# nathanweeks/exonerate

Measured on AMD Instinct MI355X. Metric: DP cells/s (first-pass lattice cells / end-to-end time), est2genome 1kb x 100kb batch, bit-exact vulgar vs reference, higher is better.
Workload: dtype int32 (packed int16 where proven exact)

## Files before the change

### exonerate_amd/csrc/c4_engine.hip

```cpp
#include <hip/hip_runtime.h>

#include <algorithm>
#include <chrono>
#include <cmath>
#include <cstdio>
#include <cstdlib>
#include <cstring>
#include <numeric>
#include <string>
#include <map>
#include <memory>
#include <vector>
#include <thread>
#include <atomic>
#include <mutex>

#include "c4gpu.h"
#include "c4_internal.h"
#include "c4_config.h"
#include "c4_memrule.h"
#include "c4_launch.h"
#include "c4_kernel_choice.h"
#include "c4_sdp_launch.h"
#include "c4_sdp_host.h"

using namespace c4k;

namespace c4h {
static thread_local std::string g_error;
void set_error(const std::string &msg) { g_error = msg; }
}

#define HIP_OK(expr)                                                                           \
    do {                                                                                       \
        hipError_t e_ = (expr);                                                                \
        if (e_ != hipSuccess) {                                                                \
            c4h::set_error(std::string(#expr) + ": " + hipGetErrorString(e_));                 \
            return -1;                                                                         \
        }                                                                                      \
    } while (0)

struct c4gpu_ctx {
    int device = 0;
    hipStream_t stream = nullptr;
    bool owns_stream = false;
// ... 25 lines not shown
```

### exonerate_amd/csrc/c4_engine_launch.inc

```
struct JobSpec {
    int pair;
    c4gpu_region region;
    int first_state = 0, final_state = 1, cp_count = 0;
    int root = 0;
    int first_cell[CELL_MAX] = {0};
    bool dump_checkpoints = false;
    const c4gpu_subopt *sub = nullptr;
    const int32_t *span_in = nullptr;
    int32_t *span_out = nullptr;
};
typedef std::vector<std::pair<int32_t, int32_t>> RegionPoints;
struct RunList {
    static constexpr int INLINE = 6;
    int n = 0;
    uint32_t small[INLINE];
    std::vector<uint32_t> big;
    const uint32_t *begin() const { return n <= INLINE ? small : big.data(); }
    const uint32_t *end() const { return begin() + n; }
    void assign_reversed(const uint32_t *first, int count) {
        n = count;
        uint32_t *dst = small;
        if (count > INLINE) { big.resize(count); dst = big.data(); }
        for (int k = 0; k < count; k++) dst[k] = first[count - 1 - k];
    }
// ... 8 lines not shown

struct SeedPlan {
    int mode = 0;
    int kshift = 11;
    bool fmt16 = false;
    int seedw = 0, dc = 0;
    std::vector<long long> off;
    std::vector<int> rows;
    std::vector<long long> base;
    std::vector<int> d, t0w, t0_base;
    int hops = 0;
};

double splice_best_sum(const c4gpu_splice_model &sp, bool absolute) {
    double sum = 0;
    for (int r = 0; r < sp.model_length && r < C4GPU_SPLICE_MAX_LEN; r++) {
        double mx = 0;
        for (int c = 0; c < 5; c++) mx = std::max(mx, absolute ? std::fabs((double)sp.data[r][c]) : (double)sp.data[r][c]);
        sum += mx;
    }
    return sum;
}

struct Engine {
    c4gpu_ctx *ctx;
    const c4gpu_model *model;
    int family;
    bool local;
    bool local_exact = true;
    bool pk16_params_ok = false;
    double calc_bound = 0;
    int pk16_match_max = 1, pk16_max_intron = 0;
    int pk16_intron_gain = 0, pk16_intron_cols = 4;
    int loop_tr_host[16] = {-1, -1, -1, -1, -1, -1, -1, -1, -1, -1, -1, -1, -1, -1, -1, -1};
    DevBuf<KParams> kparams;
    DevBuf<DevJob> d_jobs;
    DevBuf<DevResult> d_results;
    DevBuf<DevVsa> d_vsa;
    DevBuf<uint32_t> d_runs, d_runs_out;
    DevBuf<unsigned long long> d_runs_used;
    DevBuf<uint8_t> d_ops;
    DevBuf<int> d_bnd, d_ckpt, d_ckpt_dump, d_queue;
    DevBuf<uint32_t> d_tb;
    DevBuf<int> d_sub_t, d_sub_q, d_sub_colptr, d_span, d_seed, d_pairs;
    DevBuf<DevJob> d_fjobs, d_fsub_jobs;
    DevBuf<DevResult> d_fres, d_fsub_res;
    DevBuf<DevVsa> d_fvsa;
    DevBuf<int> d_ffirst, d_fflags, d_fout;
    DevBuf<unsigned long long> d_fstats;
    DevBuf<FusePair> d_fpairs;
    std::vector<DevJob> hf_jobs;
    std::vector<DevResult> hf_res;
    std::vector<int> hf_first, hf_flags, hf_out;
// ... 34 lines not shown
        }
        kp.start_scope = m->start_scope; kp.end_scope = m->end_scope;
        bool protein = false;
        for (int i = 0; i < m->n_calcs; i++)
            if (m->calcs[i].kind == C4GPU_CALC_MATCH_PROTEIN || m->calcs[i].kind == C4GPU_CALC_MATCH_P2D ||
                m->calcs[i].kind == C4GPU_CALC_MATCH_CODON) protein = true;
        memcpy(kp.submat, protein ? &params->protein_submat[0][0] : &params->dna_submat[0][0], sizeof(int) * 24 * 24);
        bool dna_match = false;
        for (int i = 0; i < m->n_calcs; i++) dna_match |= m->calcs[i].kind == C4GPU_CALC_MATCH_DNA;
        const bool veto = annotated && dna_match && !protein;
        for (int c = 0; c < 24; c++) kp.submat[24 * 24 + c] = veto ? C4GPU_IMPOSSIBLY_LOW_SCORE : 0;
        {
            double pmax = 0;
            for (int i = 0; i < m->n_calcs; i++) pmax = std::max(pmax, std::fabs((double)m->calcs[i].value));
            for (int i = 0; i < 24 * 24; i++) pmax = std::max(pmax, std::fabs((double)kp.submat[i]));
            double smax = 0;
            if (family_has_splice(family))
                for (int k = 0; k < 4; k++) smax = std::max(smax, splice_best_sum(params->splice[k], true) + 1.0);
            local_exact = (pmax + smax) * (m->n_states + 4) < 4.0e8;
            calc_bound = pmax + smax;
            double mmax = 0;
            for (int i = 0; i < 24 * 24; i++) mmax = std::max(mmax, (double)kp.submat[i]);
            pk16_match_max = (int)std::max(1.0, mmax);
            pk16_params_ok = pmax <= 16000.0 && smax <= 16000.0 && params->min_intron >= 0 && params->min_intron <= 30000 &&
                             params->max_intron >= params->min_intron;
            pk16_max_intron = params->max_intron;
            if (veto) {
                local_exact = false;
                pk16_params_ok = false;
                calc_bound = std::max(calc_bound, 987654321.0);
            }
            if (family_has_splice(family)) {
                int best[4];
                for (int k = 0; k < 4; k++) best[k] = (int)std::floor(splice_best_sum(params->splice[k], false) + 0.5) + 1;
                long long gain = -0x40000000LL;
                for (int st = 0; st < m->n_states; st++) {
                    long long pre = -0x40000000LL, post = -0x40000000LL;
                    for (int k = 0; k < m->n_transitions; k++) {
                        const c4gpu_transition &t = m->transitions[k];
                        if (t.calc < 0) continue;
                        const c4gpu_calc &cc = m->calcs[t.calc];
                        const int prm = cc.param & 3;
                        if (cc.kind == C4GPU_CALC_SPLICE_PRE && t.output == st) pre = std::max<long long>(pre, (long long)cc.value + best[prm]);
                        if (cc.kind == C4GPU_CALC_SPLICE_POST && t.input == st) post = std::max<long long>(post, (long long)cc.value + best[prm]);
                    }
                    if (pre > -0x40000000LL && post > -0x40000000LL) gain = std::max(gain, pre + post);
                }
                pk16_intron_gain = (int)std::max<long long>(0, std::min<long long>(gain, 1 << 20));
                pk16_intron_cols = std::max(4, params->min_intron);
                const bool loop_on = !(c4cfg::is(c4cfg::LOOP_SHORTCUT, 0));
                bool others_cost = true;
                for (int k = 0; k < m->n_transitions; k++) {
                    const c4gpu_transition &t = m->transitions[k];
                    if (t.advance_query != 0 || t.calc < 0) continue;
                    const c4gpu_calc &cc = m->calcs[t.calc];
                    if (cc.kind == C4GPU_CALC_SPLICE_PRE || cc.kind == C4GPU_CALC_SPLICE_POST) continue;
                    if (cc.kind != C4GPU_CALC_CONST || cc.value > 0) others_cost = false;
                }
                if (loop_on && family == FAM_EST2GENOME && others_cost && m->n_states <= 16) {
                    int tight[4];
                    for (int k = 0; k < 4; k++) tight[k] = (int)std::floor(splice_best_sum(params->splice[k], false) + 0.5 + 1e-3);
                    for (int st = 0; st < m->n_states; st++) {
                        long long pre = -0x40000000LL, post = -0x40000000LL;
                        int loop = -1;
                        bool clean = true;
                        for (int k = 0; k < m->n_transitions; k++) {
                            const c4gpu_transition &t = m->transitions[k];
                            const c4gpu_calc *cc = t.calc >= 0 ? &m->calcs[t.calc] : nullptr;
                            if (t.input == st && t.output == st) {
                                if (t.advance_query == 0 && t.advance_target == 1 && !cc && loop < 0) loop = k; else clean = false;
// ... 13 lines not shown
        }
        for (int i = 0; i < 16; i++) kp.loop_tr[i] = loop_tr_host[i];
        if (c4cfg::has(c4cfg::TRACE) && family == FAM_EST2GENOME) {
            std::string which;
            for (int i = 0; i < 16; i++) if (loop_tr_host[i] >= 0) which += " " + std::to_string(i) + ":" + std::to_string(loop_tr_host[i]);
            fprintf(stderr, "c4gpu trace: one-row sections answered without a DP for states (state:loop transition)%s\n",
                    which.empty() ? " none" : which.c_str());
        }
        for (int c = 0; c < 4096; c++) {
            const uint8_t row = params->submat_index[params->aa[params->trans[c]]];
            kp.codon_row[c] = row < 24 ? row : 0;
        }
        return 0;
    }

    bool cont_free_ok(long long q_plus_t) const {
        if (c4cfg::is(c4cfg::CONT_FREE, 0)) return false;
        return (double)(q_plus_t + 2) * std::max(calc_bound, 1.0) < 4.0e8;
    }

    bool pk16_fits(int query_length, int target_length) const {
        const double gain = (double)(query_length + 1) * pk16_match_max +
                            (double)(target_length / pk16_intron_cols + 1) * pk16_intron_gain;
        return gain <= 16000.0 && (!family_has_splice(family) || (long long)target_length + 4 <= (long long)pk16_max_intron);
    }
    int ensure_ss16(const ResidentSeqs &seqs) {
        if (!family_has_splice(family)) return 0;
        std::lock_guard<std::mutex> hold(seqs.ss16_lock);
        if (!seqs.ss16_built) {
            if (seqs.ss16.alloc((size_t)seqs.ss_len)) return -1;
            HIP_OK(pk16_build_splice(family, kparams.p, seqs.dev.ss, seqs.dev.ss_stride, seqs.ss_len, seqs.ss16.p, ctx->stream));
            HIP_OK(c4_stream_sync(ctx->stream));
            seqs.ss16_built = true;
        }
        return 0;
    }

    int run(const ResidentSeqs &seqs, int mode, bool cont, const std::vector<JobSpec> &specs, std::vector<JobOut> &out,
            SeedPlan *seed = nullptr) {
        const int n = (int)specs.size();
        if (seed) return run_impl(seqs, mode, cont, specs, out, nullptr, seed);
        for (int i = 0; i < n; i++)
            if (specs[i].span_in || specs[i].span_out) return run_impl(seqs, mode, cont, specs, out, nullptr);
        std::vector<int> plain, blocked;
        std::vector<RegionPoints> pts;
        for (int i = 0; i < n; i++) {
            const c4gpu_subopt *so = specs[i].sub ? specs[i].sub : (pair_sub ? (*pair_sub)[specs[i].pair] : nullptr);
// ... 45 lines not shown
        LaunchFacts f;
        f.family = family; f.mode = mode; f.cont = cont; f.n = n; f.blocked = pts != nullptr;
        f.local = local; f.local_exact = local_exact;
        f.starts_pack = mode == MODE_REGION;
        for (int i = 0; i < n && f.starts_pack; i++)
            f.starts_pack = nbits(specs[i].region.query_length) + nbits(specs[i].region.target_length) <= 31;
        for (int i = 0; i < n; i++) {
            const int sp = specs[i].span_in ? 1 : (specs[i].span_out ? 2 : 0);
            if (i && sp != f.span) { c4h::set_error("jobs with and without span matrices in one call"); return -1; }
            f.span = sp;
        }
        const int span = f.span;
        if (cont && (mode == MODE_PATH || mode == MODE_CKPT) && !pts && !span) {
            long long worst = 0;
            bool cells_leave = false;
            for (int i = 0; i < n; i++) {
                worst = std::max(worst, (long long)specs[i].region.query_length + specs[i].region.target_length);
                cells_leave |= specs[i].dump_checkpoints;
            }
            f.cont_free = !cells_leave && cont_free_ok(worst);
        }
        if (seed) { f.seed_mode = seed->mode; f.kshift = seed->kshift; f.fmt16 = seed->fmt16; }
        f.pk16_params_ok = pk16_params_ok;
        f.pk16_all_fit = f.seed_mode == 1;
        for (int i = 0; i < n && f.pk16_all_fit; i++) f.pk16_all_fit = pk16_fits(specs[i].region.query_length, specs[i].region.target_length);
        f.tdense_n = seqs.tdense_n; f.ss16_built = seqs.ss16_built;
        f.cu_count = ctx->prop.multiProcessorCount;
        if (!cont) {
            h_qlen.resize(n);
            for (int i = 0; i < n; i++) h_qlen[i] = specs[i].region.query_length;
            f.query_length = h_qlen.data(); f.n_lengths = n;
        }
        const KernelChoice choice = choose_kernel(f, sw);
        if (choice.error) { c4h::set_error(choice.error); return -1; }
        const KernelInfo *ki = choice.ki;
        if (choice.needs_ss16 && ensure_ss16(seqs)) return -1;
        if (seed) {
            seed->fmt16 = choice.fmt16;
            if (seed->mode == 1) { seed->seedw = ki->seedw; seed->dc = ki->max_at; }
            if (tr.on) fprintf(stderr, "c4gpu trace:   seeded pass %d with kernel %s\n", seed->mode, ki->name);
        }
        const uint8_t *staged_codes = choice.staged_codes ? seqs.tdense.p : nullptr;
        LaunchPlan lp;
        if (plan_jobs(specs, mode, ki, pts, span, seed, tr, lp)) return -1;
        if (launch_jobs(seqs, mode, ki, specs, pts, span, seed, staged_codes, tr, lp)) return -1;
        tr.lap("runs downloaded");
// ... 248 lines not shown
```

### exonerate_amd/csrc/c4_kernel_choice.h

```cpp
#pragma once
#include <algorithm>

#include "c4_config.h"
#include "c4_launch.h"

namespace c4k {

enum Pk16Form : int {
    PK16_ASM = 0,
    PK16_PLAIN = 1,
    PK16_COUNTERS = 2,
    PK16_DUMP16 = 3,
    PK16_STAGED_BARRIER = 4,
    PK16_STAGED = 5,
    PK16_STAGED_NW8 = 6,
    PK16_STAGED_R6 = 7,
    PK16_STAGED_C8 = 8,
    PK16_STAGED_LONG = 9,
    PK16_FORMS
};
enum Win16Shape : int {
    WIN16_R4W2 = 0,
    WIN16_R3W3 = 1, WIN16_R2W4 = 2, WIN16_R6W2 = 3,
    WIN16_R4W2N4 = 4,
// ... 43 lines not shown
        return s;
    }
};

struct LaunchFacts {
    int family = 0, mode = 0;
    bool cont = false;
    int n = 0;
    bool blocked = false;
    int span = 0;
    bool local = false, local_exact = false;
    bool starts_pack = false;
    bool cont_free = false;
    int seed_mode = 0;
    int kshift = 0;
    bool fmt16 = false;
    bool pk16_params_ok = false;
    bool pk16_all_fit = false;
    int tdense_n = 0;
    bool ss16_built = false;
    int cu_count = 0;
    const int *query_length = nullptr;
    int n_lengths = 0;
};

struct KernelChoice {
    const KernelInfo *ki;
    bool fmt16;
    bool needs_ss16;
    bool staged_codes;
    const char *error;
};

inline int window_waves(int family, const Switches &sw) {
    const int nw = sw.win_nw == 2 ? 2 : 4;
    return get_kernel_mw(family, MODE_REGION, true, true, nw, false, 2) ? nw : 4;
}

inline Pk16Form pk16_base_form(const Switches &sw) { return sw.pk16 == 3 ? PK16_ASM : sw.pk16 == 4 ? PK16_COUNTERS : PK16_PLAIN; }

inline bool pk16_enabled(int family, bool pk16_params_ok, long long n_jobs, const Switches &sw) {
    return family == FAM_EST2GENOME && pk16_params_ok && n_jobs >= 2 && sw.pk16 != 0 &&
           get_kernel_pk16(family, pk16_base_form(sw)) != nullptr;
}

inline void choose_pk16(const LaunchFacts &f, const Switches &sw, KernelChoice &c) {
    c.ki = get_kernel_pk16(f.family, pk16_base_form(sw));
    c.needs_ss16 = sw.pk16 != 3;
    if (sw.pk16 != 1 || !sw.win16) return;
    const KernelInfo *kd = get_kernel_pk16(f.family, PK16_DUMP16);
    if (!kd || !get_kernel_win16(f.family, WIN16_R4W2) || f.kshift > 15 || f.tdense_n <= 0) return;
    int rows = 0;
    for (int i = 0; i < f.n_lengths; i++) rows = std::max(rows, f.query_length[i] + 1);
    if (rows > 32000) return;
    c.ki = kd; c.fmt16 = true;
    const KernelInfo *ke = sw.pk16_io ? get_kernel_pk16(f.family, sw.pk16_io == 2 ? PK16_STAGED : PK16_STAGED_BARRIER) : nullptr;
    if (!ke) return;
    const bool counters = sw.pk16_io == 2;
    const bool strips_ok = rows <= pk16_staged_rows();
    if (f.tdense_n > pk16_staged_codes() && f.tdense_n <= 8 && counters && sw.pk16_c8 && strips_ok &&
        get_kernel_pk16(f.family, PK16_STAGED_C8)) {
        c.ki = get_kernel_pk16(f.family, PK16_STAGED_C8); c.staged_codes = true;
    }
    if (f.tdense_n > pk16_staged_codes()) return;
    if (strips_ok) {
        c.ki = ke; c.staged_codes = true;
        const KernelInfo *kg = (counters && sw.pk16_nw8 != 0) ? get_kernel_pk16(f.family, PK16_STAGED_NW8) : nullptr;
        if (kg && (sw.pk16_nw8 == 1 || (f.n + 1) / 2 <= f.cu_count)) c.ki = kg;
    } else if (counters && sw.pk16_r6) {
        const KernelInfo *kh = get_kernel_pk16(f.family, PK16_STAGED_R6), *kj = get_kernel_pk16(f.family, PK16_STAGED_LONG);
        if (kh && rows <= pk16_staged_rows6()) { c.ki = kh; c.staged_codes = true; }
        else if (kj && sw.pk16_long) { c.ki = kj; c.staged_codes = true; }
    }
}

inline KernelChoice choose_kernel(const LaunchFacts &f, const Switches &sw) {
    KernelChoice c{nullptr, f.fmt16, false, false, nullptr};
    const bool rect = !f.cont && (f.mode == MODE_SCORE || f.mode == MODE_REGION);
// ... 46 lines not shown
```

### exonerate_amd/csrc/c4_viterbi16_kernel.h

```cpp
#pragma once
#include "c4_viterbi_kernel.h"

namespace c4k {

typedef short pk_s2 __attribute__((ext_vector_type(2)));
template <int VAR> __device__ __forceinline__ int pk_add(int a, int b) {
    if constexpr (VAR >= 1) return __builtin_bit_cast(int, __builtin_elementwise_add_sat(__builtin_bit_cast(pk_s2, a), __builtin_bit_cast(pk_s2, b)));
    else { int r; asm("v_pk_add_i16 %0, %1, %2 clamp" : "=v"(r) : "v"(a), "v"(b)); return r; }
}
template <int VAR> __device__ __forceinline__ int pk_max(int a, int b) {
    if constexpr (VAR >= 1) return __builtin_bit_cast(int, __builtin_elementwise_max(__builtin_bit_cast(pk_s2, a), __builtin_bit_cast(pk_s2, b)));
    else { int r; asm("v_pk_max_i16 %0, %1, %2" : "=v"(r) : "v"(a), "v"(b)); return r; }
}
__device__ __forceinline__ int pk_sub(int a, int b) { int r; asm("v_pk_sub_i16 %0, %1, %2 clamp" : "=v"(r) : "v"(a), "v"(b)); return r; }
__device__ __forceinline__ int pk_neg_mask(int d, int fifteen) { int r; asm("v_pk_ashrrev_i16 %0, %1, %2" : "=v"(r) : "v"(fifteen), "v"(d)); return r; }
template <int VAR> __device__ __forceinline__ int pk_lt_mask(int a, int b, int fifteen) {
    if constexpr (VAR >= 1) {
        int r;
        asm("v_pk_sub_i16 %0, %1, %2 clamp\n\tv_pk_ashrrev_i16 %0, 15, %0 op_sel_hi:[0,1]" : "=&v"(r) : "v"(a), "v"(b));
        return r;
    } else {
        return pk_neg_mask(pk_sub(a, b), fifteen);
    }
}
__device__ __forceinline__ int pk_pack(int lo, int hi) { return (int)__builtin_amdgcn_perm((unsigned)hi, (unsigned)lo, 0x05040100u); }
__device__ __forceinline__ int pk_half(int x, int h) { return h ? (x >> 16) : ((x << 16) >> 16); }
__device__ __forceinline__ int clamp16(int x) { return x < -32768 ? -32768 : (x > 32767 ? 32767 : x); }

constexpr int NEG16 = (int)0x80008000u;


template <class M>
struct Dump16 {
    using W1 = WaveDP<M, 1, MODE_SCORE, false, true, false, false, 0, 1>;
    static constexpr bool live(int s) { return M::NDES > 0 && W1::slot_live(s, 0); }
    static constexpr bool inner(int s) { return s != M::START && s != M::END; }
    static constexpr int n_inner() { int n = 0; for (int s = 0; s < M::NS; s++) n += inner(s); return n; }
    static constexpr int n_live() { int n = 0; for (int s = 0; s < M::NS; s++) n += (inner(s) && live(s)); return n; }
    static constexpr int NH = n_inner() + n_live();
    static constexpr int SEEDW16 = (NH + 1) / 2;
    static constexpr int half_of_sc(int s) { int n = 0; for (int x = 0; x < s; x++) n += inner(x); return n; }
    static constexpr int half_of_il(int s) { int n = n_inner(); for (int x = 0; x < s; x++) n += (inner(x) && live(x)); return n; }
    static constexpr int state_of_half(int h) {
        if (h < n_inner()) { for (int s = 0; s < M::NS; s++) if (inner(s) && half_of_sc(s) == h) return s; return -1; }
        for (int s = 0; s < M::NS; s++) if (inner(s) && live(s) && half_of_il(s) == h) return s;
        return -1;
    }
};

template <class M, int R, int VAR = 0, bool DUMP16 = false, int IO = 0, int NCODE_ = 6, bool MEMC = false>
struct WaveDP16 {
    using F = Facts<M>;
    static_assert(M::MAXAQ == 1, "the packed forms exchange exactly one query row per step");
    using W32 = WaveDP<M, R, MODE_SCORE, false, true, false, false, 0, 1>;
    using D16 = Dump16<M>;
    static constexpr int NS = M::NS, NCOL = M::MAXAT + 1, W = 64 * R, DC = M::MAXAT, SEEDW = DUMP16 ? D16::SEEDW16 : W32::SEEDW;
    static constexpr bool live(int s) { return M::NDES > 0 && W32::slot_live(s, 0); }
    static constexpr int NEXP = F::n_exported();
    static constexpr int n_exported_live() { int n = 0; for (int x = 0; x < NS; x++) n += (F::exported(x) && live(x)); return n; }
    static constexpr int BND = IO ? (NEXP + n_exported_live() + 3) / 4 * 4 : NEXP * 2;
    static constexpr int RING = 256;
    static constexpr int CH = IO ? 63 / NCOL * NCOL : (64 + NCOL - 1) / NCOL * NCOL;
    static constexpr int NCODE = NCODE_;
    static constexpr int STAGE_COLS = 128, STAGE_INTS = 8;
    static constexpr int NP = (R + 1) / 2, PROF_EB = (R == 6) ? 12 : 8, PROF_CODE = 64 * PROF_EB;
    static constexpr int PROF_INTS = NCODE * PROF_CODE / 4;
    static_assert(!IO || (VAR >= 1 && F::has_splice() && (R == 6 || R == 4 || R == 2)), "the staged form is built for the packed splice entries and 2, 4 or 6 rows per lane");
    static_assert(!F::has_phase(), "split-codon calcs are not packed");
    static_assert(M::NDES <= 1, "one shadow designation");
    typedef __attribute__((address_space(3))) int lds_int;
    struct C16 { int sc[NS]; int il[NS]; };
    __device__ __forceinline__ static lds_int *lds_at(int a) { return (lds_int *)(size_t)(unsigned)a; }
    __device__ __forceinline__ static int lds_addr(const lds_int *p) { return (int)(unsigned)(size_t)p; }

    const KParams *kp;
    int lane;
    const uint8_t *qc[2], *tc[2];
    const int *ss[2];
    const uint2 *ss16[2];
    long long ss_stride;
// ... 79 lines not shown
    __device__ __forceinline__ void prefetch_profile() {
        const lds_int *pa = lds_at(prof_a[0] + nx_off[0]), *pb = lds_at(prof_a[1] + nx_off[1]);
        static_for<NP>([&](auto K_) __attribute__((always_inline)) { constexpr int K = K_; nx_prof[K] = pa[K]; nx_prof[3 + K] = pb[K]; });
    }
    __device__ __forceinline__ void fill_stage(lds_int *stage, int c0) {
        constexpr int mat = F::match_at();
        const int c = c0 + lane;
        uint2 sv[2]; int off[2];
        static_for<2>([&](auto H_) __attribute__((always_inline)) { constexpr int H = H_;
            int ti = t0[H] + c - mat;
            ti = ti < 0 ? 0 : (ti > tlast[H] ? tlast[H] : ti);
            int tp = t0[H] + c - 2;
            tp = tp < 0 ? 0 : (tp > tlast[H] ? tlast[H] : tp);
            sv[H] = ss16[H][(unsigned)tp];
            off[H] = (int)tdense[tc[H][(unsigned)ti]] * PROF_CODE;
        });
        lds_int *p = stage + (c & (STAGE_COLS - 1));
        p[0 * STAGE_COLS] = (int)__builtin_amdgcn_perm(sv[1].x, sv[0].x, 0x05040100u);
        p[1 * STAGE_COLS] = (int)__builtin_amdgcn_perm(sv[1].x, sv[0].x, 0x07060302u);
        p[2 * STAGE_COLS] = (int)__builtin_amdgcn_perm(sv[1].y, sv[0].y, 0x05040100u);
        p[3 * STAGE_COLS] = (int)__builtin_amdgcn_perm(sv[1].y, sv[0].y, 0x07060302u);
        p[4 * STAGE_COLS] = off[0]; p[5 * STAGE_COLS] = off[1];
    }
    static constexpr int DEAD_ROW = -16000;
    __device__ __forceinline__ void build_profile(int i0) {
        static_for<2>([&](auto H_) __attribute__((always_inline)) { constexpr int H = H_;
            int qr[R];
            static_for<R>([&](auto RR_) __attribute__((always_inline)) { constexpr int RR = RR_;
                const int i = i0 + RR;
                qr[RR] = 24 * ((i >= 1 && i <= Q[H]) ? (int)qc[H][q0[H] + i - 1] : 0);
            });
            for (int d = 0; d < NCODE; d++) {
                const int code = tdense[24 + d];
                int v[R];
                static_for<R>([&](auto RR_) __attribute__((always_inline)) { constexpr int RR = RR_;
                    v[RR] = (i0 + RR > Q[H]) ? DEAD_ROW : clamp16(kp->submat[qr[RR] + code]);
                });
                lds_int *p = lds_at(prof_a[H] + d * PROF_CODE);
                static_for<NP>([&](auto K_) __attribute__((always_inline)) { constexpr int K = K_; p[K] = pk_pack(v[2 * K], v[2 * K + 1 < R ? 2 * K + 1 : 2 * K]); });
            }
        });
    }

    __device__ __forceinline__ void prefetch_column(int j) {
        if constexpr (IO == 1) { prefetch_staged(); return; }
        constexpr int mat = F::match_at();
        static_for<2>([&](auto H_) __attribute__((always_inline)) { constexpr int H = H_;
            int ti = t0[H] + j - mat;
            ti = ti < 0 ? 0 : (ti > tlast[H] ? tlast[H] : ti);
            nx_tcode[H] = tc[H][(unsigned)ti];
            if constexpr (F::has_splice()) {
                int tp = t0[H] + j - 2;
                tp = tp < 0 ? 0 : (tp > tlast[H] ? tlast[H] : tp);
                if constexpr (VAR >= 1) {
                    nx_sp16[H] = ss16[H][(unsigned)tp];
                } else {
                    static_for<4>([&](auto K_) __attribute__((always_inline)) { constexpr int K = K_;
                        nx_sp[H][K] = ss[H][(long long)K * ss_stride + tp];
                    });
                }
            }
        });
    }

    template <int RR, int PH, bool JINT>
    __device__ __forceinline__ void eval_cell(int j, int ms, const int (&sp)[4]) {
        C16 &c = col[PH][RR];
        static_for<M::NT>([&](auto K_) __attribute__((always_inline)) { constexpr int K = K_;
            constexpr TrDesc t = M::tr[K];
            constexpr int PD = (PH - t.at + NCOL) % NCOL;
            const C16 &src = (t.aq == 0) ? col[PD][RR] : (RR > 0 ? col[PD][RR > 0 ? RR - 1 : 0] : nbr[PD]);
            int cand;
            if constexpr (t.in == M::START) cand = 0;
            else cand = src.sc[t.in];
            if constexpr (t.calc >= 0) {
                constexpr CalcDesc cd = M::calc[t.calc];
                if constexpr (cd.kind == CALC_CONST) cand = pk_add<VAR>(cand, cv_pk[t.calc]);
                else if constexpr (cd.kind >= CALC_MATCH_DNA && cd.kind <= CALC_MATCH_P2D) cand = pk_add<VAR>(cand, ms);
                else if constexpr (cd.kind == CALC_SPLICE_PRE) cand = pk_add<VAR>(cand, sp[cd.param]);
                else if constexpr (cd.kind == CALC_SPLICE_POST) {
                    static_assert(live(t.in), "post-splice calc without a length");
                    const int bad = pk_neg_mask(src.il[t.in], fifteen);
                    const int sv = (bad & NEG16) | (~bad & sp[cd.param]);
                    cand = pk_add<VAR>(cand, sv);
                }
            }
            if constexpr (!JINT && t.at > 0) cand = (j >= t.at) ? cand : NEG16;
            int ilc = 0;
            if constexpr (live(t.out)) {
                if constexpr (F::owns_shadow(t.in, 0)) ilc = open_il_pk;
                else if constexpr (live(t.in)) ilc = pk_add<VAR>(src.il[t.in], at_pk[t.at]);
            }
            if constexpr (F::code(K) == 1) {
                c.sc[t.out] = cand;
                if constexpr (live(t.out)) c.il[t.out] = ilc;
            } else {
                if constexpr (live(t.out)) {
                    const int win = pk_lt_mask<VAR>(c.sc[t.out], cand, fifteen);
                    c.il[t.out] = (win & ilc) | (~win & c.il[t.out]);
                }
                c.sc[t.out] = pk_max<VAR>(c.sc[t.out], cand);
            }
        });
    }

    template <bool JINT, int PH>
    __device__ __forceinline__ void step(int s, int i0, bool last_strip, const int *bnd_in, int *bnd_out) {
        const int j = s - lane;
        int ms[R];
        if constexpr (IO == 1) {
            static_for<NP>([&](auto K_) __attribute__((always_inline)) { constexpr int K = K_;
                ms[2 * K] = (int)__builtin_amdgcn_perm((unsigned)nx_prof[3 + K], (unsigned)nx_prof[K], 0x05040100u);
                if constexpr (2 * K + 1 < R) ms[2 * K + 1] = (int)__builtin_amdgcn_perm((unsigned)nx_prof[3 + K], (unsigned)nx_prof[K], 0x07060302u);
            });
        } else {
            static_for<R>([&](auto RR_) __attribute__((always_inline)) { constexpr int RR = RR_;
                ms[RR] = pk_pack(kp->submat[qrow[0][RR] + nx_tcode[0]], kp->submat[qrow[1][RR] + nx_tcode[1]]);
            });
// ... 6 lines not shown
            sp[1] = (int)__builtin_amdgcn_perm(nx_sp16[1].x, nx_sp16[0].x, 0x07060302u);
            sp[2] = (int)__builtin_amdgcn_perm(nx_sp16[1].y, nx_sp16[0].y, 0x05040100u);
            sp[3] = (int)__builtin_amdgcn_perm(nx_sp16[1].y, nx_sp16[0].y, 0x07060302u);
        } else if constexpr (F::has_splice()) {
            static_for<M::NC>([&](auto CI_) __attribute__((always_inline)) { constexpr int CI = CI_;
                constexpr CalcDesc cd = M::calc[CI];
                if constexpr (cd.kind == CALC_SPLICE_PRE)
                    sp[cd.param] = pk_pack(clamp16(kp->calc_value[CI] + nx_sp[0][cd.param]), clamp16(kp->calc_value[CI] + nx_sp[1][cd.param]));
                if constexpr (cd.kind == CALC_SPLICE_POST)
                    sp[cd.param] = pk_pack(clamp16(nx_sp[0][cd.param]), clamp16(nx_sp[1][cd.param]));
            });
        }
        for_exported([&](auto S_, int) __attribute__((always_inline)) { constexpr int S = S_;
            nbr[PH].sc[S] = dpp_shr1(nx_carry.sc[S], expo.sc[S]);
            if constexpr (live(S)) nbr[PH].il[S] = dpp_shr1(nx_carry.il[S], expo.il[S]);
        });
        prefetch_carry(s + 1, bnd_in);
        prefetch_column(j + 1);
        static_for<R>([&](auto RR_) __attribute__((always_inline)) { constexpr int RR = RR_;
            eval_cell<RR, PH, JINT>(j, ms[RR], sp);
            if constexpr (IO == 1 && RR == R / 2 - 1) prefetch_profile();
        });
        {
            int m = col[PH][0].sc[M::END];
            static_for<R>([&](auto RR_) __attribute__((always_inline)) { constexpr int RR = RR_; if constexpr (RR > 0) m = pk_max<VAR>(m, col[PH][RR].sc[M::END]); });
            const bool cand = (pk_sub(best_pk, m) & NEG16) != 0;
            if (__builtin_amdgcn_ballot_w64(cand)) {
                static_for<2>([&](auto H_) __attribute__((always_inline)) { constexpr int H = H_;
                    const bool jact = (j >= 0) & (j <= T[H]);
                    static_for<R>([&](auto RR_) __attribute__((always_inline)) { constexpr int RR = RR_;
                        const int tsc = pk_half(col[PH][RR].sc[M::END], H);
                        const bool upd = jact & (i0 + RR <= Q[H]) & (!best_set[H] | (best[H] < tsc));
                        int from = -1, fsc = 0;
                        static_for<M::NT>([&](auto K_) __attribute__((always_inline)) { constexpr int K = K_;
                            constexpr TrDesc t = M::tr[K];
                            if constexpr (t.out == M::END && t.in != M::START) {
                                const int v = pk_half(col[PH][RR].sc[t.in], H);
                                const bool win = (from < 0) | (fsc < v);
                                fsc = win ? v : fsc;
                                from = win ? t.in : from;
                            }
                        });
                        best[H] = upd ? tsc : best[H];
                        best_i[H] = upd ? (((i0 + RR) << 4) | from) : best_i[H];
                        best_j[H] = upd ? j : best_j[H];
                        best_set[H] = best_set[H] | upd;
                    });
                });
                best_pk = pk_pack(best_set[0] ? best[0] : pk_half(unset_pk, 0), best_set[1] ? best[1] : pk_half(unset_pk, 1));
            }
        }
        for_exported([&](auto S_, int) __attribute__((always_inline)) { constexpr int S = S_;
            expo.sc[S] = col[PH][R - 1].sc[S];
            if constexpr (live(S)) expo.il[S] = col[PH][R - 1].il[S];
        });
        if constexpr (IO == 1) {
            if (lane == 63 && (JINT || (j >= 0 && j <= Tm))) {
                bool to_memory = false;
                if constexpr (MEMC) to_memory = mem_out;
                if (to_memory) {
                    int *p = bnd_out + (long long)j * BND;
                    for_exported([&](auto S_, int slot) __attribute__((always_inline)) { constexpr int S = S_;
                        p[slot] = expo.sc[S];
                        if constexpr (live(S)) p[slot + 1] = expo.il[S];
                    });
                } else {
                    lds_int *p = ring_out + (j & ring_out_mask) * BND;
                    for_exported([&](auto S_, int slot) __attribute__((always_inline)) { constexpr int S = S_;
                        p[slot] = expo.sc[S];
                        if constexpr (live(S)) p[slot + 1] = expo.il[S];
                    });
                }
// ... 6 lines not shown
                    if constexpr (live(S)) p[1] = expo.il[S];
                });
            } else {
                for_exported([&](auto S_, int slot) __attribute__((always_inline)) { constexpr int S = S_;
                    int *p = bnd_out + (long long)j * BND + slot;
                    p[0] = expo.sc[S];
                    if constexpr (live(S)) p[1] = expo.il[S];
                });
            }
        }
        if (((unsigned)(s + DC - 1) & (unsigned)((1 << seed_kshift) - 1)) <= (unsigned)(DC + 62)) {
            const int d = (j + DC - 1) >> seed_kshift;
            const unsigned which = (unsigned)(j - ((d << seed_kshift) - (DC - 1)));
            static_for<2>([&](auto H_) __attribute__((always_inline)) { constexpr int H = H_;
                if ((j >= 0) & (j <= T[H]) & (d >= 1) & (which < (unsigned)DC) & ((d << seed_kshift) <= T[H])) {
                    static_for<R>([&](auto RR_) __attribute__((always_inline)) { constexpr int RR = RR_;
                        const int i = i0 + RR;
                        if (i <= Q[H]) {
                            int *p = seed_wr[H] + (((long long)(d - 1) * DC + which) * seed_rows[H] + i) * SEEDW;
                            if constexpr (DUMP16) {
                                auto half_reg = [&](auto HI_) __attribute__((always_inline)) -> int { constexpr int HI = HI_;
                                    constexpr int S = D16::state_of_half(HI);
                                    if constexpr (S < 0) return 0;
                                    else if constexpr (HI < D16::n_inner()) return col[PH][RR].sc[S];
                                    else return pk_add<VAR>(col[PH][RR].il[S], lim_pk);
                                };
                                static_for<D16::SEEDW16>([&](auto K_) __attribute__((always_inline)) { constexpr int K = K_;
                                    const int va = half_reg(IC<2 * K>{}), vb = half_reg(IC<2 * K + 1>{});
                                    store_dword<K * 4>(p, (int)__builtin_amdgcn_perm((unsigned)vb, (unsigned)va, H ? 0x07060302u : 0x05040100u));
                                });
                            } else {
                                static_for<NS>([&](auto S_) __attribute__((always_inline)) { constexpr int S = S_;
                                    store_dword<S * 4>(p, pk_half(col[PH][RR].sc[S], H));
                                    if constexpr (live(S))
                                        store_dword<W32::dump_pos(S, 0) * 4>(p, t0[H] + j - pk_half(pk_add<VAR>(col[PH][RR].il[S], lim_pk), H) - 2);
                                });
                            }
                        }
                    });
                }
            });
        }
    }

    __device__ __forceinline__ void strip_begin() {
        static_for<2>([&](auto H_) __attribute__((always_inline)) { constexpr int H = H_;
            sbest[H] = best[H]; sbest_i[H] = best_i[H]; sbest_j[H] = best_j[H]; sbest_set[H] = best_set[H];
// ... 163 lines not shown
            strip_end();
            __builtin_amdgcn_fence(__ATOMIC_RELEASE, "workgroup");
            __syncthreads();
        }
    }
};

template <class M>
__global__ void ss16_kernel(const KParams *kp, const int *ss, long long ss_stride, long long n, uint2 *out) {
    for (long long p = (long long)blockIdx.x * blockDim.x + threadIdx.x; p < n; p += (long long)gridDim.x * blockDim.x) {
        int v[4] = {0, 0, 0, 0};
        static_for<M::NC>([&](auto CI_) __attribute__((always_inline)) { constexpr int CI = CI_;
            constexpr CalcDesc cd = M::calc[CI];
            if constexpr (cd.kind == CALC_SPLICE_PRE) v[cd.param] = clamp16(kp->calc_value[CI] + ss[cd.param * ss_stride + p]);
            if constexpr (cd.kind == CALC_SPLICE_POST) v[cd.param] = clamp16(ss[cd.param * ss_stride + p]);
        });
        uint2 o;
        o.x = ((unsigned)v[0] & 0xffffu) | ((unsigned)v[1] << 16);
        o.y = ((unsigned)v[2] & 0xffffu) | ((unsigned)v[3] << 16);
        out[p] = o;
    }
}

template <class M, int R, int NW, int WPE, int VAR = 0, bool DUMP16 = false, int IO = 0, int NCODE_ = 6, bool MEMC = false>
__global__ __launch_bounds__(64 * NW) __attribute__((amdgpu_waves_per_eu(WPE, 8)))
void viterbi16_kernel_mw(const KParams *kparams, DevSeqs seqs, const DevJob *jobs, int n_jobs, DevResult *results,
                         DevScratch scratch, int *queue, const uint8_t *tdense = nullptr) {
    using DP = WaveDP16<M, R, VAR, DUMP16, IO, NCODE_, MEMC>;
    __shared__ __attribute__((aligned(4096))) int stage_mem[IO ? NW * DP::STAGE_COLS * DP::STAGE_INTS : 1];
    __shared__ __attribute__((aligned(16))) int prof_mem[IO ? NW * 2 * DP::PROF_INTS : 1];
    __shared__ __attribute__((aligned(16))) int edge_cols[IO ? 2 * DP::BND : 1];
    __shared__ __attribute__((aligned(16))) int kp_stage[IO ? 1 : (sizeof(KParams) + 3) / 4];
    __shared__ int next_job;
    __shared__ __attribute__((aligned(16))) int rings[(NW > 1 ? NW - 1 : 1) * DP::RING * DP::BND];
    __shared__ int wave_best[NW][2][4];
    __shared__ int progress[NW];
    if constexpr (IO == 0) {
        const int *src = reinterpret_cast<const int *>(kparams);
        int *dst = kp_stage;
        for (int x = threadIdx.x; x < (int)(sizeof(KParams) / sizeof(int)); x += 64 * NW) dst[x] = src[x];
    } else {
        if (threadIdx.x == 0) DP::write_empty_column((typename DP::lds_int *)edge_cols);
    }
    __syncthreads();
    const int wid = __builtin_amdgcn_readfirstlane(threadIdx.x >> 6);
    int *bnd = scratch.bnd + (long long)blockIdx.x * scratch.bnd_stride;
    if (threadIdx.x == 0) DP::write_empty_column(bnd);
    __builtin_amdgcn_fence(__ATOMIC_RELEASE, "workgroup");
    __syncthreads();
    const int n_pairs = (n_jobs + 1) / 2;
    for (;;) {
// ... 52 lines not shown
```

### exonerate_amd/csrc/kernels/kpk16_families.hip

```cpp
#include "../c4_kernel_choice.h"
#include "../c4_viterbi16_kernel.h"
namespace c4k {
template <class M, int R, int NW, int WPE, int VAR, bool D16, int IO = 0, int NCODE = 6, bool MEMC = false>
struct Pk16 {
    using DP = WaveDP16<M, R, VAR, D16, IO, NCODE, MEMC>;
    static constexpr auto kernel = viterbi16_kernel_mw<M, R, NW, WPE, VAR, D16, IO, NCODE, MEMC>;
    static hipError_t launch(const LaunchArgs &a) {
        hipLaunchKernelGGL(kernel, dim3(a.grid), dim3(64 * NW), 0, a.stream, a.kp, a.seqs, a.jobs, a.n_jobs, a.results, a.scratch,
                           a.queue, IO ? reinterpret_cast<const uint8_t *>(a.aux) : nullptr);
        return hipGetLastError();
    }
    static KernelInfo info(const char *name) {
        return {launch, (const void *)kernel, name, R, 2, DP::BND, M::NS, M::MAXAT, NW, DP::SEEDW};
    }
};
using E = Est2GenomeDesc;
static const KernelInfo pk16_forms[PK16_FORMS] = {
    Pk16<E, 4, 4, 3, 0, false>::info("kpk16_est2genome"),
    Pk16<E, 4, 4, 3, 1, false>::info("kpk16b_est2genome"),
    Pk16<E, 4, 4, 3, 2, false>::info("kpk16c_est2genome"),
    Pk16<E, 4, 4, 3, 1, true>::info("kpk16d_est2genome"),
    Pk16<E, 4, 4, 3, 1, true, 1>::info("kpk16e_est2genome"),
    Pk16<E, 4, 4, 3, 2, true, 1>::info("kpk16f_est2genome"),
    Pk16<E, 2, 8, 2, 2, true, 1>::info("kpk16g_est2genome"),
    Pk16<E, 6, 4, 2, 2, true, 1>::info("kpk16h_est2genome"),
    Pk16<E, 4, 4, 2, 2, true, 1, 8>::info("kpk16i_est2genome"),
    Pk16<E, 6, 4, 2, 2, true, 1, 6, true>::info("kpk16j_est2genome"),
};
static int rows_of(Pk16Form f) { return pk16_forms[f].R * 64 * pk16_forms[f].waves; }
// ... 14 lines not shown
```

Baseline: 1038 billion.

## Bias packed int16 scores so fp16 max3 folds three-way state maxima

Staged packed-16 kernels now store every score offset by a constant bias so that legitimate values are positive finite fp16 bit patterns. Because positive fp16 values order the same way as their int16 bit patterns, a single packed half max3 can replace two int16 max operations for non-live states with three or more incoming transitions. END is no longer computed per transition and is instead taken as a max3 reduction over the states that feed it. Dumps and best-score bookkeeping subtract the bias again. A host-side check on the substitution, calc and splice bounds falls back to the unbiased path when parameters could leave the exact range, which adds more exactness-sensitive code.

```diff
diff --git a/exonerate_amd/csrc/c4_engine.hip b/exonerate_amd/csrc/c4_engine.hip
--- a/exonerate_amd/csrc/c4_engine.hip
+++ b/exonerate_amd/csrc/c4_engine.hip
@@ -21,6 +21,7 @@
 #include "c4_memrule.h"
 #include "c4_launch.h"
 #include "c4_kernel_choice.h"
+#include "c4_pk16_bias.h"
 #include "c4_sdp_launch.h"
 #include "c4_sdp_host.h"
 
diff --git a/exonerate_amd/csrc/c4_engine_launch.inc b/exonerate_amd/csrc/c4_engine_launch.inc
--- a/exonerate_amd/csrc/c4_engine_launch.inc
+++ b/exonerate_amd/csrc/c4_engine_launch.inc
@@ -54,6 +54,16 @@
     return sum;
 }
 
+double splice_worst_sum(const c4gpu_splice_model &sp) {
+    double sum = 0;
+    for (int r = 0; r < sp.model_length && r < C4GPU_SPLICE_MAX_LEN; r++) {
+        double mn = 0;
+        for (int c = 0; c < 5; c++) mn = std::min(mn, (double)sp.data[r][c]);
+        sum += mn;
+    }
+    return sum;
+}
+
 struct Engine {
     c4gpu_ctx *ctx;
     const c4gpu_model *model;
@@ -61,6 +71,7 @@
     bool local;
     bool local_exact = true;
     bool pk16_params_ok = false;
+    bool pk16_bias_ok = false;
     double calc_bound = 0;
     int pk16_match_max = 1, pk16_max_intron = 0;
     int pk16_intron_gain = 0, pk16_intron_cols = 4;
@@ -141,9 +152,10 @@
             double mmax = 0;
             for (int i = 0; i < 24 * 24; i++) mmax = std::max(mmax, (double)kp.submat[i]);
             pk16_match_max = (int)std::max(1.0, mmax);
-            pk16_params_ok = pmax <= 16000.0 && smax <= 16000.0 && params->min_intron >= 0 && params->min_intron <= 30000 &&
+            pk16_params_ok = pmax <= (double)PK16_SCORE_MAX && smax <= (double)PK16_SCORE_MAX && params->min_intron >= 0 && params->min_intron <= 30000 &&
                              params->max_intron >= params->min_intron;
             pk16_max_intron = params->max_intron;
+            pk16_bias_ok = false;
             if (veto) {
                 local_exact = false;
                 pk16_params_ok = false;
@@ -165,6 +177,18 @@
                     }
                     if (pre > -0x40000000LL && post > -0x40000000LL) gain = std::max(gain, pre + post);
                 }
+                long long site_worst[4] = {0, 0, 0, 0}, post_best = 0;
+                for (int i = 0; i < m->n_calcs; i++) {
+                    const c4gpu_calc &cc = m->calcs[i];
+                    const int prm = cc.param & 3;
+                    const long long worst = (long long)std::floor(splice_worst_sum(params->splice[prm]) - 0.5) - 1;
+                    if (cc.kind == C4GPU_CALC_SPLICE_PRE) site_worst[prm] = std::min(site_worst[prm], (long long)cc.value + worst);
+                    if (cc.kind == C4GPU_CALC_SPLICE_POST) {
+                        site_worst[prm] = std::min(site_worst[prm], worst);
+                        post_best = std::max<long long>(post_best, best[prm]);
+                    }
+                }
+                pk16_bias_ok = pk16_bias_fits(kp.submat, 24 * 24, kp.calc_value, m->n_calcs, site_worst, 4, post_best);
                 pk16_intron_gain = (int)std::max<long long>(0, std::min<long long>(gain, 1 << 20));
                 pk16_intron_cols = std::max(4, params->min_intron);
                 const bool loop_on = !(c4cfg::is(c4cfg::LOOP_SHORTCUT, 0));
@@ -224,7 +248,7 @@
     bool pk16_fits(int query_length, int target_length) const {
         const double gain = (double)(query_length + 1) * pk16_match_max +
                             (double)(target_length / pk16_intron_cols + 1) * pk16_intron_gain;
-        return gain <= 16000.0 && (!family_has_splice(family) || (long long)target_length + 4 <= (long long)pk16_max_intron);
+        return gain <= (double)PK16_SCORE_MAX && (!family_has_splice(family) || (long long)target_length + 4 <= (long long)pk16_max_intron);
     }
     int ensure_ss16(const ResidentSeqs &seqs) {
         if (!family_has_splice(family)) return 0;
@@ -316,6 +340,7 @@
         }
         if (seed) { f.seed_mode = seed->mode; f.kshift = seed->kshift; f.fmt16 = seed->fmt16; }
         f.pk16_params_ok = pk16_params_ok;
+        f.pk16_bias_unfit = !pk16_bias_ok;
         f.pk16_all_fit = f.seed_mode == 1;
         for (int i = 0; i < n && f.pk16_all_fit; i++) f.pk16_all_fit = pk16_fits(specs[i].region.query_length, specs[i].region.target_length);
         f.tdense_n = seqs.tdense_n; f.ss16_built = seqs.ss16_built;
diff --git a/exonerate_amd/csrc/c4_kernel_choice.h b/exonerate_amd/csrc/c4_kernel_choice.h
--- a/exonerate_amd/csrc/c4_kernel_choice.h
+++ b/exonerate_amd/csrc/c4_kernel_choice.h
@@ -89,6 +89,7 @@
     int cu_count = 0;
     const int *query_length = nullptr;
     int n_lengths = 0;
+    bool pk16_bias_unfit = false;
 };
 
 struct KernelChoice {
@@ -121,6 +122,7 @@
     for (int i = 0; i < f.n_lengths; i++) rows = std::max(rows, f.query_length[i] + 1);
     if (rows > 32000) return;
     c.ki = kd; c.fmt16 = true;
+    if (f.pk16_bias_unfit) return;
     const KernelInfo *ke = sw.pk16_io ? get_kernel_pk16(f.family, sw.pk16_io == 2 ? PK16_STAGED : PK16_STAGED_BARRIER) : nullptr;
     if (!ke) return;
     const bool counters = sw.pk16_io == 2;
diff --git a/exonerate_amd/csrc/c4_pk16_bias.h b/exonerate_amd/csrc/c4_pk16_bias.h
--- /dev/null
+++ b/exonerate_amd/csrc/c4_pk16_bias.h
@@ -0,0 +1,28 @@
+#pragma once
+
+namespace c4k {
+
+constexpr int PK16_SCORE_MAX = 16000;
+constexpr int PK16_HALF_FINITE_MAX = 0x7BFF;
+constexpr int PK16_HALF_NORMAL_MIN = 0x0400;
+constexpr int PK16_POST_GAIN_MAX = 127;
+constexpr int PK16_BIAS = PK16_HALF_FINITE_MAX - PK16_SCORE_MAX - PK16_POST_GAIN_MAX;
+constexpr int PK16_ADDEND_MAX = (PK16_BIAS - PK16_HALF_NORMAL_MIN) / 2;
+static_assert(PK16_BIAS + PK16_SCORE_MAX + PK16_POST_GAIN_MAX <= PK16_HALF_FINITE_MAX, "the largest legitimate half is finite");
+static_assert(PK16_BIAS - 2 * PK16_ADDEND_MAX >= PK16_HALF_NORMAL_MIN, "the smallest legitimate candidate is a normal half");
+static_assert(PK16_HALF_FINITE_MAX - 32768 == -1025 && -1025 < -1024, "legitimate + (-32 768) is a negative finite half (0xFBFF at most)");
+static_assert(-32768 + PK16_SCORE_MAX + PK16_POST_GAIN_MAX < -1024, "the lineage of `unset` stays a negative finite half");
+
+inline bool pk16_bias_addend_ok(long long v) { return v >= -(long long)PK16_ADDEND_MAX || v <= -32768; }
+
+inline bool pk16_bias_site_ok(long long worst_sum) { return worst_sum >= -(long long)PK16_ADDEND_MAX; }
+
+inline bool pk16_bias_fits(const int *submat, int n_submat, const int *calc_value, int n_calcs, const long long *site_worst,
+                           int n_sites, long long post_best) {
+    for (int i = 0; i < n_submat; i++) if (!pk16_bias_addend_ok(submat[i])) return false;
+    for (int i = 0; i < n_calcs; i++) if (!pk16_bias_addend_ok(calc_value[i])) return false;
+    for (int i = 0; i < n_sites; i++) if (!pk16_bias_site_ok(site_worst[i])) return false;
+    return post_best <= PK16_POST_GAIN_MAX;
+}
+
+}
diff --git a/exonerate_amd/csrc/c4_viterbi16_kernel.h b/exonerate_amd/csrc/c4_viterbi16_kernel.h
--- a/exonerate_amd/csrc/c4_viterbi16_kernel.h
+++ b/exonerate_amd/csrc/c4_viterbi16_kernel.h
@@ -1,4 +1,5 @@
 #pragma once
+#include "c4_pk16_bias.h"
 #include "c4_viterbi_kernel.h"
 
 namespace c4k {
@@ -11,6 +12,11 @@
 template <int VAR> __device__ __forceinline__ int pk_max(int a, int b) {
     if constexpr (VAR >= 1) return __builtin_bit_cast(int, __builtin_elementwise_max(__builtin_bit_cast(pk_s2, a), __builtin_bit_cast(pk_s2, b)));
     else { int r; asm("v_pk_max_i16 %0, %1, %2" : "=v"(r) : "v"(a), "v"(b)); return r; }
+}
+typedef _Float16 pk_h2 __attribute__((ext_vector_type(2)));
+__device__ __forceinline__ int pk_max3(int a, int b, int c) {
+    return __builtin_bit_cast(int, __builtin_elementwise_maximum(__builtin_elementwise_maximum(__builtin_bit_cast(pk_h2, a), __builtin_bit_cast(pk_h2, b)),
+                                                                 __builtin_bit_cast(pk_h2, c)));
 }
 __device__ __forceinline__ int pk_sub(int a, int b) { int r; asm("v_pk_sub_i16 %0, %1, %2 clamp" : "=v"(r) : "v"(a), "v"(b)); return r; }
 __device__ __forceinline__ int pk_neg_mask(int d, int fifteen) { int r; asm("v_pk_ashrrev_i16 %0, %1, %2" : "=v"(r) : "v"(fifteen), "v"(d)); return r; }
@@ -48,14 +54,25 @@
     }
 };
 
-template <class M, int R, int VAR = 0, bool DUMP16 = false, int IO = 0, int NCODE_ = 6, bool MEMC = false>
+template <class M, int R, int VAR = 0, bool DUMP16 = false, int IO = 0, int NCODE_ = 6, bool MEMC = false, bool BIAS = false>
 struct WaveDP16 {
     using F = Facts<M>;
+    static_assert(!BIAS || (IO == 1 && DUMP16), "the biased form is the staged one: dead rows by the profile, 16-bit dumps");
+    static constexpr int B_PK = BIAS ? PK16_BIAS * 0x10001 : 0;
     static_assert(M::MAXAQ == 1, "the packed forms exchange exactly one query row per step");
     using W32 = WaveDP<M, R, MODE_SCORE, false, true, false, false, 0, 1>;
     using D16 = Dump16<M>;
     static constexpr int NS = M::NS, NCOL = M::MAXAT + 1, W = 64 * R, DC = M::MAXAT, SEEDW = DUMP16 ? D16::SEEDW16 : W32::SEEDW;
     static constexpr bool live(int s) { return M::NDES > 0 && W32::slot_live(s, 0); }
+    static constexpr int n_into(int s) { int n = 0; for (int k = 0; k < M::NT; k++) n += (M::tr[k].out == s); return n; }
+    static constexpr bool max3_state(int s) { return BIAS && s != M::END && !live(s) && n_into(s) >= 3; }
+    static constexpr bool feeds_end(int s) { for (int k = 0; k < M::NT; k++) if (M::tr[k].out == M::END && M::tr[k].in == s) return true; return false; }
+    static_assert(!BIAS || !feeds_end(M::START), "END's value is the maximum of inner states");
+    static constexpr bool end_is_plain_max() {
+        for (int k = 0; k < M::NT; k++) if (M::tr[k].out == M::END && (M::tr[k].aq != 0 || M::tr[k].at != 0 || M::tr[k].calc >= 0)) return false;
+        return true;
+    }
+    static_assert(!BIAS || end_is_plain_max(), "the biased form takes END as the plain maximum of the states that enter it");
     static constexpr int NEXP = F::n_exported();
     static constexpr int n_exported_live() { int n = 0; for (int x = 0; x < NS; x++) n += (F::exported(x) && live(x)); return n; }
     static constexpr int BND = IO ? (NEXP + n_exported_live() + 3) / 4 * 4 : NEXP * 2;
@@ -181,7 +198,7 @@
         p[3 * STAGE_COLS] = (int)__builtin_amdgcn_perm(sv[1].y, sv[0].y, 0x07060302u);
         p[4 * STAGE_COLS] = off[0]; p[5 * STAGE_COLS] = off[1];
     }
-    static constexpr int DEAD_ROW = -16000;
+    static constexpr int DEAD_ROW = BIAS ? -32768 : -16000;
     __device__ __forceinline__ void build_profile(int i0) {
         static_for<2>([&](auto H_) __attribute__((always_inline)) { constexpr int H = H_;
             int qr[R];
@@ -225,12 +242,14 @@
     template <int RR, int PH, bool JINT>
     __device__ __forceinline__ void eval_cell(int j, int ms, const int (&sp)[4]) {
         C16 &c = col[PH][RR];
+        int pend[NS];
         static_for<M::NT>([&](auto K_) __attribute__((always_inline)) { constexpr int K = K_;
             constexpr TrDesc t = M::tr[K];
+            if constexpr (BIAS && t.out == M::END) return;
             constexpr int PD = (PH - t.at + NCOL) % NCOL;
             const C16 &src = (t.aq == 0) ? col[PD][RR] : (RR > 0 ? col[PD][RR > 0 ? RR - 1 : 0] : nbr[PD]);
             int cand;
-            if constexpr (t.in == M::START) cand = 0;
+            if constexpr (t.in == M::START) cand = B_PK;
             else cand = src.sc[t.in];
             if constexpr (t.calc >= 0) {
                 constexpr CalcDesc cd = M::calc[t.calc];
@@ -253,6 +272,11 @@
             if constexpr (F::code(K) == 1) {
                 c.sc[t.out] = cand;
                 if constexpr (live(t.out)) c.il[t.out] = ilc;
+            } else if constexpr (max3_state(t.out)) {
+                constexpr int nth = F::code(K) - 1;
+                if constexpr (nth % 2 == 0) c.sc[t.out] = pk_max3(c.sc[t.out], pend[t.out], cand);
+                else if constexpr (nth + 1 < n_into(t.out)) pend[t.out] = cand;
+                else c.sc[t.out] = pk_max<VAR>(c.sc[t.out], cand);
             } else {
                 if constexpr (live(t.out)) {
                     const int win = pk_lt_mask<VAR>(c.sc[t.out], cand, fifteen);
@@ -305,15 +329,30 @@
             if constexpr (IO == 1 && RR == R / 2 - 1) prefetch_profile();
         });
         {
-            int m = col[PH][0].sc[M::END];
-            static_for<R>([&](auto RR_) __attribute__((always_inline)) { constexpr int RR = RR_; if constexpr (RR > 0) m = pk_max<VAR>(m, col[PH][RR].sc[M::END]); });
+            int m = 0;
+            if constexpr (BIAS) {
+                int pend = 0, n = 0;
+                static_for<R>([&](auto RR_) __attribute__((always_inline)) { constexpr int RR = RR_;
+                    static_for<NS>([&](auto S_) __attribute__((always_inline)) { constexpr int S = S_;
+                        if constexpr (feeds_end(S)) {
+                            const int v = col[PH][RR].sc[S];
+                            if (n == 0) m = v;
+                            else if (n % 2 == 1) pend = v;
+                            else m = pk_max3(m, pend, v);
+                            n++;
+                        }
+                    });
+                });
+                if (n % 2 == 0) m = pk_max<VAR>(m, pend);
+            } else {
+                m = col[PH][0].sc[M::END];
+                static_for<R>([&](auto RR_) __attribute__((always_inline)) { constexpr int RR = RR_; if constexpr (RR > 0) m = pk_max<VAR>(m, col[PH][RR].sc[M::END]); });
+            }
             const bool cand = (pk_sub(best_pk, m) & NEG16) != 0;
             if (__builtin_amdgcn_ballot_w64(cand)) {
                 static_for<2>([&](auto H_) __attribute__((always_inline)) { constexpr int H = H_;
                     const bool jact = (j >= 0) & (j <= T[H]);
                     static_for<R>([&](auto RR_) __attribute__((always_inline)) { constexpr int RR = RR_;
-                        const int tsc = pk_half(col[PH][RR].sc[M::END], H);
-                        const bool upd = jact & (i0 + RR <= Q[H]) & (!best_set[H] | (best[H] < tsc));
                         int from = -1, fsc = 0;
                         static_for<M::NT>([&](auto K_) __attribute__((always_inline)) { constexpr int K = K_;
                             constexpr TrDesc t = M::tr[K];
@@ -324,13 +363,16 @@
                                 from = win ? t.in : from;
                             }
                         });
+                        const int tsc = BIAS ? fsc - PK16_BIAS : pk_half(col[PH][RR].sc[M::END], H);
+                        const bool upd = jact & (i0 + RR <= Q[H]) & (!best_set[H] | (best[H] < tsc));
                         best[H] = upd ? tsc : best[H];
                         best_i[H] = upd ? (((i0 + RR) << 4) | from) : best_i[H];
                         best_j[H] = upd ? j : best_j[H];
                         best_set[H] = best_set[H] | upd;
                     });
                 });
-                best_pk = pk_pack(best_set[0] ? best[0] : pk_half(unset_pk, 0), best_set[1] ? best[1] : pk_half(unset_pk, 1));
+                constexpr int B = BIAS ? PK16_BIAS : 0;
+                best_pk = pk_pack(best_set[0] ? best[0] + B : pk_half(unset_pk, 0), best_set[1] ? best[1] + B : pk_half(unset_pk, 1));
             }
         }
         for_exported([&](auto S_, int) __attribute__((always_inline)) { constexpr int S = S_;
@@ -383,7 +425,10 @@
                                 auto half_reg = [&](auto HI_) __attribute__((always_inline)) -> int { constexpr int HI = HI_;
                                     constexpr int S = D16::state_of_half(HI);
                                     if constexpr (S < 0) return 0;
-                                    else if constexpr (HI < D16::n_inner()) return col[PH][RR].sc[S];
+                                    else if constexpr (HI < D16::n_inner()) {
+                                        if constexpr (BIAS) return pk_sub(col[PH][RR].sc[S], B_PK);
+                                        else return col[PH][RR].sc[S];
+                                    }
                                     else return pk_add<VAR>(col[PH][RR].il[S], lim_pk);
                                 };
                                 static_for<D16::SEEDW16>([&](auto K_) __attribute__((always_inline)) { constexpr int K = K_;
@@ -593,11 +638,11 @@
     }
 }
 
-template <class M, int R, int NW, int WPE, int VAR = 0, bool DUMP16 = false, int IO = 0, int NCODE_ = 6, bool MEMC = false>
+template <class M, int R, int NW, int WPE, int VAR = 0, bool DUMP16 = false, int IO = 0, int NCODE_ = 6, bool MEMC = false, bool BIAS = false>
 __global__ __launch_bounds__(64 * NW) __attribute__((amdgpu_waves_per_eu(WPE, 8)))
 void viterbi16_kernel_mw(const KParams *kparams, DevSeqs seqs, const DevJob *jobs, int n_jobs, DevResult *results,
                          DevScratch scratch, int *queue, const uint8_t *tdense = nullptr) {
-    using DP = WaveDP16<M, R, VAR, DUMP16, IO, NCODE_, MEMC>;
+    using DP = WaveDP16<M, R, VAR, DUMP16, IO, NCODE_, MEMC, BIAS>;
     __shared__ __attribute__((aligned(4096))) int stage_mem[IO ? NW * DP::STAGE_COLS * DP::STAGE_INTS : 1];
     __shared__ __attribute__((aligned(16))) int prof_mem[IO ? NW * 2 * DP::PROF_INTS : 1];
     __shared__ __attribute__((aligned(16))) int edge_cols[IO ? 2 * DP::BND : 1];
diff --git a/exonerate_amd/csrc/kernels/kpk16_families.hip b/exonerate_amd/csrc/kernels/kpk16_families.hip
--- a/exonerate_amd/csrc/kernels/kpk16_families.hip
+++ b/exonerate_amd/csrc/kernels/kpk16_families.hip
@@ -3,8 +3,8 @@
 namespace c4k {
 template <class M, int R, int NW, int WPE, int VAR, bool D16, int IO = 0, int NCODE = 6, bool MEMC = false>
 struct Pk16 {
-    using DP = WaveDP16<M, R, VAR, D16, IO, NCODE, MEMC>;
-    static constexpr auto kernel = viterbi16_kernel_mw<M, R, NW, WPE, VAR, D16, IO, NCODE, MEMC>;
+    using DP = WaveDP16<M, R, VAR, D16, IO, NCODE, MEMC, IO == 1>;
+    static constexpr auto kernel = viterbi16_kernel_mw<M, R, NW, WPE, VAR, D16, IO, NCODE, MEMC, IO == 1>;
     static hipError_t launch(const LaunchArgs &a) {
         hipLaunchKernelGGL(kernel, dim3(a.grid), dim3(64 * NW), 0, a.stream, a.kp, a.seqs, a.jobs, a.n_jobs, a.results, a.scratch,
                            a.queue, IO ? reinterpret_cast<const uint8_t *>(a.aux) : nullptr);
```

New measurement: 1094 billion, median of 6. 5.5% higher.
